# kylejckson/PaintFE

Hardware: AMD Instinct MI355X
Metric: Mpixels/sec: 8K 32-layer flatten + Gaussian sigma=16; HBM GB/s vs peak (higher is better)
Workload: dtype f32 (Gaussian leg: f16 taps x u8, f32 accumulate)

## Files before the change

paintfe_amd/csrc/k_flatten.hip:

```cpp
#include <algorithm>
#include <atomic>
#include <type_traits>
#include "k_common.h"
#include "pfx_kernels.h"

using namespace pfxk;

#include "k_blend.h"

typedef float pfx_v4f __attribute__((ext_vector_type(4)));
typedef int pfx_v4i __attribute__((ext_vector_type(4)));
__device__ pfx_v4f pfx_buffer_load_format_v4f32(pfx_v4i rsrc, int voffset, int soffset, int aux) __asm("llvm.amdgcn.raw.buffer.load.format.v4f32");
__device__ float pfx_buffer_load_format_f32(pfx_v4i rsrc, int voffset, int soffset, int aux) __asm("llvm.amdgcn.raw.buffer.load.format.f32");
__device__ void pfx_buffer_store_i32(int data, pfx_v4i rsrc, int voffset, int soffset, int aux) __asm("llvm.amdgcn.raw.buffer.store.i32");
__device__ void pfx_buffer_store_format_v4f32(pfx_v4f data, pfx_v4i rsrc, int voffset, int soffset, int aux) __asm("llvm.amdgcn.raw.buffer.store.format.v4f32");


namespace {


PFX_DEV uint32_t apply_conceal(uint32_t px, uint32_t conceal)
{
    if (conceal == 0u) return px;
    uint32_t a = ((px >> 24) * (255u - conceal)) / 255u;
// ... 417 lines not shown
                            const float a = pfx_buffer_load_format_f32(ra, (int)((base_px + o0 + 64u * j) * 4u), 0, 0);
                            const bool hit = C.kind[i] ? (a == 1.0f) : (a != 0.0f);
                            cls[j] = (cls[j] == 0u && hit) ? (uint32_t)(i + 1) : cls[j];
                            all_found = all_found && cls[j] != 0u;
                        }
                        done = __all(all_found);
                        st_reads += 1u;
                    }
                }
                uint32_t cnt[5] = {UPX, 0u, 0u, 0u, 0u};
#pragma unroll
                for (int i = 1; i <= 4; ++i)
#pragma unroll
                    for (int j = 0; j < PX; ++j) cnt[i] += (uint32_t)__popcll(__ballot(cls[j] >= (uint32_t)i));
                uint32_t cmin = 0;
#pragma unroll
                for (int i = 1; i <= 4; ++i) if (cnt[i] == UPX) cmin = (uint32_t)i;
                uint32_t lay[5] = {0u, C.layer[0], C.layer[1], C.layer[2], C.layer[3]};
                uint32_t s_u = 0;
#pragma unroll
                for (int i = 1; i <= 4; ++i) if (cmin == (uint32_t)i) s_u = lay[i];
                uint32_t best = 0, best_sav = 0, r = s_u;
#pragma unroll
                for (int i = 1; i <= 4; ++i) {
                    if ((uint32_t)i > cmin && (uint32_t)i <= C.n && cnt[i] * 10u >= UPX * 3u) {
                        const uint32_t sav = cnt[i] * (lay[i] - s_u);
                        if (sav > best_sav) { best_sav = sav; best = (uint32_t)i; r = lay[i]; }
                    }
                }
                if (best != 0u && q_cnt != 0u && q_r != r) { best = 0u; r = s_u; }
                if (probe) {
                    if (best != 0u || s_u != 0u) probe_fail = 0u;
                    else if (++probe_fail >= 2u) { probe_fail = 0u; skip_left = 14u; }
                }
#pragma unroll
                for (int j = 0; j < PX; ++j) acc_ring[(o0 + 64u * j) % RING] = 0u;
                if (best != 0u) {
                    st_cunits += 1u;
                    if (q_cnt == 0u) q_start = s_u; else q_start = min(q_start, s_u);
                    q_r = r;
#pragma unroll
                    for (int j = 0; j < PX; ++j) {
                        const bool early = cls[j] < best;
                        const uint64_t m = __ballot(early);
                        const uint32_t pre = __builtin_amdgcn_mbcnt_hi((uint32_t)(m >> 32), __builtin_amdgcn_mbcnt_lo((uint32_t)m, 0u));
                        if (early) q[(q_tail + pre) % QCAP] = (uint16_t)(o0 + 64u * j);
                        q_tail += (uint32_t)__popcll(m);
                    }
                }
                if (lane == 0) { rec[u % NREC][0] = r; rec[u % NREC][1] = best != 0u ? q_tail : 0u; }
                wave_lds_sync();
                cls_next = u + 1u;
                continue;
            }
            if (q_cnt == 0u) {
                if (lane == 0 && (C.stats & 1u)) {
                    atomicAdd(&g_dle_stats[0], st_rounds); atomicAdd(&g_dle_stats[1], st_rpx); atomicAdd(&g_dle_stats[2], st_rlay);
                    atomicAdd(&g_dle_stats[3], nat_next); atomicAdd(&g_dle_stats[4], st_nlay); atomicAdd(&g_dle_stats[5], st_reads);
                    atomicAdd(&g_dle_stats[6], st_cunits);
                }
                break;
            }
            run_queue = true;
        }

        int voff[PX];
        float acc[PX][4];
        uint32_t lb, le;
        if (run_queue) {
            const uint32_t m = min(q_cnt, UPX);
#pragma unroll
            for (int j = 0; j < PX; ++j) {
                const uint32_t k = 64u * j + lane;
                const uint32_t o = (uint32_t)q[(q_head + k) % QCAP];
                voff[j] = k < m ? (int)((base_px + o) * 4u) : (int)bytes;
                acc[j][0] = acc[j][1] = acc[j][2] = acc[j][3] = 0.0f;
            }
            lb = q_start; le = q_r;
            q_head += m;
            st_rounds += 1u; st_rpx += m; st_rlay += le - lb;
        } else {
            const uint32_t o0 = nat_next * UPX + lane;
#pragma unroll
            for (int j = 0; j < PX; ++j) {
                voff[j] = (int)((base_px + o0 + 64u * j) * 4u);
                const uint32_t p = acc_ring[(o0 + 64u * j) % RING];
                acc[j][0] = div255(ubyte0(p)); acc[j][1] = div255(ubyte1(p)); acc[j][2] = div255(ubyte2(p)); acc[j][3] = div255(ubyte3(p));
            }
            lb = nat_start; le = n_layers;
            st_nlay += le - lb;
        }
        dle_layers<PX, NB, AUX>(acc, layers, lb, le, bytes, voff, (C.stats & 2u) != 0u);
#pragma unroll
        for (int j = 0; j < PX; ++j) {
            const uint32_t px = (uint32_t)(acc[j][0] * 255.0f + 0.5f) | ((uint32_t)(acc[j][1] * 255.0f + 0.5f) << 8) |
                                ((uint32_t)(acc[j][2] * 255.0f + 0.5f) << 16) | ((uint32_t)(acc[j][3] * 255.0f + 0.5f) << 24);
            if (run_queue) { if (voff[j] != (int)bytes) acc_ring[((uint32_t)voff[j] / 4u - base_px) % RING] = px; }
            else pfx_buffer_store_i32((int)px, rs_dst, voff[j], 0, 0);
        }
        if (run_queue) wave_lds_sync();
        else nat_next += 1u;
    }
}


#ifndef PFX_SRT_GROUPS
#define PFX_SRT_GROUPS 1
#endif
#ifndef PFX_SRT_REDEAL
#define PFX_SRT_REDEAL 1
#endif
#ifndef PFX_SRT_TYPED_STORE
#define PFX_SRT_TYPED_STORE 0
#endif
#ifndef PFX_SRT_NATSTORE
#define PFX_SRT_NATSTORE 1
#endif
template <int PX>
PFX_DEV void stream_layer_groups(float (&acc)[PX][4], const float (&t)[PX][4], uint32_t mode, float opacity, uint32_t lead)
{
    const float amax = alpha_max<PX>(t);
#if PFX_TWO_STAGE
    if (__any(amax != 0.0f)) blend_layer_nx_two_stage<PX>(mode, acc, t, opacity, lead);
#elif PFX_SRT_GROUPS
    if (__any(amax != 0.0f)) blend_layer_nx_groups<PX>(mode, acc, t, opacity, lead);
#else
    if (__any(amax != 0.0f)) blend_layer_nx<PX>(mode, acc, t, opacity);
#endif
}

template <int PX, bool NOBLEND = false, bool TR = false>
PFX_DEV void srt_layers(float (&acc)[PX][4], const pfxk_layer_desc* __restrict__ layers, uint32_t lb, uint32_t le, uint32_t bytes, int (&voff)[PX],
                        uint32_t s1, uint32_t seg, float4* s_x, uint32_t* s_v, uint32_t& st_moves, unsigned long long* tr = nullptr)
{
    float t[2][PX][4];
    uint32_t m[2], o[2];
    const pfxk_layer_desc* nptr = layers + lb;
    pfxk_layer_desc nd = *nptr;
    uint32_t next_attempt = lb < s1 ? s1 : lb + 1u;
    uint32_t lead = 0u;
    bool recount = true;
    auto fetch = [&](auto SET) {
        constexpr int S = decltype(SET)::value;
        m[S] = nd.mode; o[S] = nd.adj_off;
        const pfx_v4i rs = make_rsrc_canonical(nd.pixels, bytes, PFX_RSRC_UNORM8X4);
#pragma unroll
        for (int j = 0; j < PX; ++j) {
            const pfx_v4f v = pfx_buffer_load_format_v4f32(rs, voff[j], 0, 0);
            t[S][j][0] = v.x; t[S][j][1] = v.y; t[S][j][2] = v.z; t[S][j][3] = v.w;
        }
        nptr += 1;
        nd = *nptr;
    };
    auto blend = [&](auto SET, uint32_t K) {
        constexpr int S = decltype(SET)::value;
        if (K < le) {
            unsigned long long c0 = 0, c1 = 0;
            if constexpr (TR) {
                c0 = __builtin_amdgcn_s_memtime();
                if constexpr (PX == 1) asm volatile("s_waitcnt vmcnt(1)" ::: "memory");
                else if constexpr (PX == 2) asm volatile("s_waitcnt vmcnt(2)" ::: "memory");
                else asm volatile("s_waitcnt vmcnt(3)" ::: "memory");
                c1 = __builtin_amdgcn_s_memtime();
                tr[0] += c1 - c0;
            }
            if constexpr (NOBLEND) {
#pragma unroll
                for (int j = 0; j < PX; ++j) { acc[j][0] += t[S][j][0]; acc[j][1] += t[S][j][1]; acc[j][2] += t[S][j][2]; acc[j][3] = t[S][j][3]; }
            } else if constexpr (PX == 1 && !PFX_TWO_STAGE) {
                stream_layer<1>(acc, t[S], m[S], __builtin_bit_cast(float, __builtin_amdgcn_readfirstlane(o[S])));
            } else {
                if (recount) { lead = count_lead<PX>(acc); recount = false; }
                stream_layer_groups<PX>(acc, t[S], m[S], __builtin_bit_cast(float, __builtin_amdgcn_readfirstlane(o[S])), lead);
                recount = m[S] == M_XOR || m[S] == M_OVERWRITE;
            }
            if constexpr (TR) {
                float sink = 0.0f;
#pragma unroll
                for (int j = 0; j < PX; ++j) sink += acc[j][0] + acc[j][3];
                asm volatile("" :: "v"(sink));
                tr[1] += __builtin_amdgcn_s_memtime() - c1;
            }
        }
    };
    auto redeal = [&](auto SET, uint32_t K) {
        constexpr int S = decltype(SET)::value;
#if !PFX_SRT_REDEAL
        return;
#endif
        if constexpr (PX == 1 || NOBLEND) return;
        if (K != next_attempt || K >= le) return;
        next_attempt = K + seg;
        uint64_t mo[PX];
        uint32_t co[PX], total_o = 0u, now = 0u;
        bool run = true;
#pragma unroll
        for (int j = 0; j < PX; ++j) {
            mo[j] = __ballot(acc[j][3] == 1.0f);
            co[j] = (uint32_t)__popcll(mo[j]);
            total_o += co[j];
            run = run && co[j] == 64u;
            now += run ? 1u : 0u;
        }
        lead = now; recount = false;
        if (total_o / 64u <= now) return;
        lead = total_o / 64u;
        const uint32_t lane = __builtin_amdgcn_mbcnt_hi(~0u, __builtin_amdgcn_mbcnt_lo(~0u, 0u));
        uint32_t slot[PX], pre_o = 0u, pre_n = total_o;
#pragma unroll
        for (int j = 0; j < PX; ++j) {
            const uint32_t rank_o = __builtin_amdgcn_mbcnt_hi((uint32_t)(mo[j] >> 32), __builtin_amdgcn_mbcnt_lo((uint32_t)mo[j], 0u));
            slot[j] = acc[j][3] == 1.0f ? pre_o + rank_o : pre_n + (lane - rank_o);
            pre_o += co[j]; pre_n += 64u - co[j];
        }
#pragma unroll
        for (int j = 0; j < PX; ++j) { s_x[slot[j]] = make_float4(acc[j][0], acc[j][1], acc[j][2], acc[j][3]); s_v[slot[j]] = (uint32_t)voff[j]; }
        wave_lds_sync();
#pragma unroll
        for (int j = 0; j < PX; ++j) {
            const float4 a = s_x[64u * j + lane];
            acc[j][0] = a.x; acc[j][1] = a.y; acc[j][2] = a.z; acc[j][3] = a.w;
            voff[j] = (int)s_v[64u * j + lane];
        }
        wave_lds_sync();
#pragma unroll
        for (int j = 0; j < PX; ++j) s_x[slot[j]] = make_float4(t[S][j][0], t[S][j][1], t[S][j][2], t[S][j][3]);
        wave_lds_sync();
#pragma unroll
        for (int j = 0; j < PX; ++j) {
            const float4 a = s_x[64u * j + lane];
            t[S][j][0] = a.x; t[S][j][1] = a.y; t[S][j][2] = a.z; t[S][j][3] = a.w;
        }
        wave_lds_sync();
        st_moves += 1u;
    };
    fetch(std::integral_constant<int, 0>{});
    for (uint32_t li = lb; li < le; li += 2) {
        fetch(std::integral_constant<int, 1>{}); blend(std::integral_constant<int, 0>{}, li); redeal(std::integral_constant<int, 1>{}, li + 1);
        fetch(std::integral_constant<int, 0>{}); blend(std::integral_constant<int, 1>{}, li + 1); redeal(std::integral_constant<int, 0>{}, li + 2);
    }
}

template <int NB, bool NOBLEND = false, bool TR = false>
PFX_DEV void srt_early(float (&acc)[1][4], const pfxk_layer_desc* __restrict__ layers, uint32_t lb, uint32_t le, uint32_t bytes, int voff, unsigned long long* tr = nullptr)
{
    static_assert(NB >= 2 && 2 * NB - 2 < PFXK_DESC_PAD, "descriptor padding");
    float t[NB][1][4];
    uint32_t m[NB], o[NB];
    const pfxk_layer_desc* nptr = layers + lb;
    pfxk_layer_desc nd = *nptr;
    uint32_t lead = 0u;
    bool recount = true;
    auto fetch = [&](auto SET) {
        constexpr int S = decltype(SET)::value;
        m[S] = nd.mode; o[S] = nd.adj_off;
        const pfx_v4i rs = make_rsrc_canonical(nd.pixels, bytes, PFX_RSRC_UNORM8X4);
        const pfx_v4f v = pfx_buffer_load_format_v4f32(rs, voff, 0, 0);
        t[S][0][0] = v.x; t[S][0][1] = v.y; t[S][0][2] = v.z; t[S][0][3] = v.w;
        nptr += 1;
        nd = *nptr;
    };
    auto blend = [&](auto SET, uint32_t K) {
        constexpr int S = decltype(SET)::value;
        if (K < le) {
            unsigned long long c0 = 0, c1 = 0;
            if constexpr (TR) {
                c0 = __builtin_amdgcn_s_memtime();
                asm volatile("s_waitcnt vmcnt(%0)" :: "n"(NB - 1) : "memory");
                c1 = __builtin_amdgcn_s_memtime();
                tr[0] += c1 - c0;
            }
            if constexpr (NOBLEND) { acc[0][0] += t[S][0][0]; acc[0][1] += t[S][0][1]; acc[0][2] += t[S][0][2]; acc[0][3] = t[S][0][3]; }
            else {
                if (recount) { lead = count_lead<1>(acc); recount = false; }
                stream_layer_groups<1>(acc, t[S], m[S], __builtin_bit_cast(float, __builtin_amdgcn_readfirstlane(o[S])), lead);
                recount = true;
            }
            if constexpr (TR) {
                const float sink = acc[0][0] + acc[0][3];
                asm volatile("" :: "v"(sink));
                tr[1] += __builtin_amdgcn_s_memtime() - c1;
            }
        }
    };
    auto seq = [&](auto self, auto I, uint32_t li) {
        constexpr int i = decltype(I)::value;
        if constexpr (i < NB) {
            fetch(std::integral_constant<int, (i + NB - 1) % NB>{});
            blend(std::integral_constant<int, i>{}, li + (uint32_t)i);
            self(self, std::integral_constant<int, i + 1>{}, li);
        }
    };
    auto pre = [&](auto self, auto I) {
        constexpr int i = decltype(I)::value;
        if constexpr (i < NB - 1) { fetch(std::integral_constant<int, i>{}); self(self, std::integral_constant<int, i + 1>{}); }
    };
    pre(pre, std::integral_constant<int, 0>{});
    for (uint32_t li = lb; li < le; li += (uint32_t)NB) seq(seq, std::integral_constant<int, 0>{}, li);
}
#ifndef PFX_EARLY_NB
#define PFX_EARLY_NB 2
#endif

struct dle_plan { uint32_t s1, seg; };

#ifndef PFX_SRT_PRIO
#define PFX_SRT_PRIO 0
#endif
#ifndef PFX_SRT_WAVES
#define PFX_SRT_WAVES 8
#endif
#if PFX_SRT_WAVES == 8
#define PFX_SRT_ATTR __attribute__((amdgpu_waves_per_eu(8, 8)))
#elif PFX_SRT_WAVES == 7
#define PFX_SRT_ATTR __attribute__((amdgpu_waves_per_eu(7, 7)))
#else
#define PFX_SRT_ATTR
#endif
template <int PX, bool NOBLEND = false, bool TR = false>
__global__ __launch_bounds__(64) PFX_SRT_ATTR void flatten_srt_kernel(const pfxk_layer_desc* __restrict__ layers, uint32_t n_layers, uint32_t n_px,
                                                                         uint8_t* __restrict__ dst, const pfxk_dle_cands C, const dle_sched SC,
                                                                         const dle_plan P)
{
    constexpr uint32_t UPX = 64u * PX;
    __shared__ float4 s_x[UPX];
    __shared__ uint32_t s_v[UPX];
    soft_d_fill(threadIdx.x, 64u);
    __syncthreads();
    const uint32_t lane = threadIdx.x & 63u;
    const uint32_t gw = __builtin_amdgcn_readfirstlane(blockIdx.x);
    const uint32_t units_total = (n_px + UPX - 1u) / UPX;
    uint32_t u0, U;
    if (gw < SC.wavesA) { U = SC.UA; u0 = gw * SC.UA; }
    else if (gw < SC.wavesA + SC.wavesB) { U = SC.UB; u0 = SC.wavesA * SC.UA + (gw - SC.wavesA) * SC.UB; }
    else { U = SC.UC; u0 = SC.wavesA * SC.UA + SC.wavesB * SC.UB + (gw - SC.wavesA - SC.wavesB) * SC.UC; }
    if (u0 >= units_total) return;
    const uint32_t nu = min(U, units_total - u0);
    const uint32_t base_px = u0 * UPX;
    const uint32_t bytes = n_px * 4u;
#if PFX_SRT_TYPED_STORE
    const pfx_v4i rs_acc = make_rsrc(dst, bytes, PFX_RSRC_UNORM8X4);
#else
    const pfx_v4i rs_dst = make_rsrc(dst, bytes, PFX_RSRC_RAW32);
#endif
    const uint32_t s1 = P.seg != 0u ? P.s1 : 0xFFFFFFFFu;
    uint32_t st_egroups = 0, st_elay = 0, st_nlay = 0, st_reads = 0, st_cunits = 0, st_moves = 0;
    uint32_t probe_fail = 0, skip_left = 0;
    unsigned long long tph[8] = {0, 0, 0, 0, 0, 0, 0, 0}, tc0 = 0;
    const unsigned long long t_birth = TR ? __builtin_amdgcn_s_memtime() : 0ull;
    for (uint32_t u = 0; u < nu; ++u) {
        if constexpr (TR) tc0 = __builtin_amdgcn_s_memtime();
        int voff[PX];
        float acc[PX][4];
#pragma unroll
        for (int j = 0; j < PX; ++j) {
            voff[j] = (int)((base_px + u * UPX + 64u * j + lane) * 4u);
            acc[j][0] = acc[j][1] = acc[j][2] = acc[j][3] = 0.0f;
        }
        uint32_t cls[PX];
#pragma unroll
        for (int j = 0; j < PX; ++j) cls[j] = 0u;
        const bool probe = skip_left == 0u;
        if (!probe) skip_left -= 1u;
        bool done = !probe;
#pragma unroll
        for (int i = 3; i >= 0; --i) {
            if ((uint32_t)i < C.n && !done) {
                const pfx_v4i ra = make_rsrc(layers[C.layer[i]].pixels, bytes, PFX_RSRC_ALPHA8);
                bool all_found = true;
#pragma unroll
                for (int j = 0; j < PX; ++j) {
                    const float a = pfx_buffer_load_format_f32(ra, voff[j], 0, 0);
                    const bool hit = C.kind[i] ? (a == 1.0f) : (a != 0.0f);
                    cls[j] = (cls[j] == 0u && hit) ? (uint32_t)(i + 1) : cls[j];
                    all_found = all_found && cls[j] != 0u;
                }
                done = __all(all_found);
                st_reads += 1u;
            }
        }
        uint32_t cn[5] = {UPX, 0u, 0u, 0u, 0u};
#pragma unroll
        for (int i = 1; i <= 4; ++i)
#pragma unroll
            for (int j = 0; j < PX; ++j) cn[i] += (uint32_t)__popcll(__ballot(cls[j] >= (uint32_t)i));
        uint32_t cmin = 0;
#pragma unroll
        for (int i = 1; i <= 4; ++i) if (cn[i] == UPX) cmin = (uint32_t)i;
        const uint32_t lay[5] = {0u, C.layer[0], C.layer[1], C.layer[2], C.layer[3]};
        uint32_t s_u = 0;
#pragma unroll
        for (int i = 1; i <= 4; ++i) if (cmin == (uint32_t)i) s_u = lay[i];
        uint32_t best = 0, best_sav = 0, r = s_u, eg = 0, cn_best = 0;
#pragma unroll
        for (int i = 1; i <= 4; ++i) {
            if ((uint32_t)i > cmin && (uint32_t)i <= C.n) {
                const uint32_t g = (UPX - cn[i] + 63u) / 64u;
                const uint32_t sav = ((uint32_t)PX - g) * (lay[i] - s_u);
                if (sav > best_sav) { best_sav = sav; best = (uint32_t)i; r = lay[i]; eg = g; cn_best = cn[i]; }
            }
        }
        if (probe) {
            if (best != 0u || s_u != 0u) probe_fail = 0u;
            else if (++probe_fail >= 2u) { probe_fail = 0u; skip_left = 14u; }
        }
        if constexpr (TR) { const unsigned long long c = __builtin_amdgcn_s_memtime(); tph[0] += c - tc0; tc0 = c; }
        if (best != 0u) {
            st_cunits += 1u;
            uint32_t pre_e = 0u, pre_l = UPX - cn_best;
#pragma unroll
            for (int j = 0; j < PX; ++j) {
                const bool early = cls[j] < best;
                const uint64_t m = __ballot(early);
                const uint32_t rank_e = __builtin_amdgcn_mbcnt_hi((uint32_t)(m >> 32), __builtin_amdgcn_mbcnt_lo((uint32_t)m, 0u));
                const uint32_t c = (uint32_t)__popcll(m);
                s_v[early ? pre_e + rank_e : pre_l + (lane - rank_e)] = (uint32_t)voff[j];
                pre_e += c; pre_l += 64u - c;
            }
            wave_lds_sync();
#pragma unroll
            for (int j = 0; j < PX; ++j) voff[j] = (int)s_v[64u * j + lane];
            wave_lds_sync();
            for (uint32_t g = 0; g < eg; ++g) {
                int v1[1];
                float a1[1][4] = {{0.0f, 0.0f, 0.0f, 0.0f}};
                v1[0] = voff[0];
#pragma unroll
                for (int j = 1; j < PX; ++j) v1[0] = g == (uint32_t)j ? voff[j] : v1[0];
                uint32_t none = 0u;
#if PFX_SRT_PRIO
                __builtin_amdgcn_s_setprio(PFX_SRT_PRIO & 3);
#endif
#if PFX_EARLY_NB > 0
                (void)none;
                srt_early<PFX_EARLY_NB, NOBLEND, TR>(a1, layers, s_u, r, bytes, v1[0], tph + 4);
#else
                srt_layers<1, NOBLEND, TR>(a1, layers, s_u, r, bytes, v1, 0xFFFFFFFFu, 0u, s_x, s_v, none, tph + 4);
#endif
#pragma unroll
                for (int j = 0; j < PX; ++j)
                    if (g == (uint32_t)j) { acc[j][0] = a1[0][0]; acc[j][1] = a1[0][1]; acc[j][2] = a1[0][2]; acc[j][3] = a1[0][3]; }
            }
            st_egroups += eg; st_elay += eg * (r - s_u);
        }
        st_nlay += n_layers - r;
        const uint32_t moves_before = st_moves;
        if constexpr (TR) { const unsigned long long c = __builtin_amdgcn_s_memtime(); tph[1] += c - tc0; tc0 = c; }
#if PFX_SRT_PRIO
        __builtin_amdgcn_s_setprio((PFX_SRT_PRIO >> 2) & 3);
#endif
        srt_layers<PX, NOBLEND, TR>(acc, layers, r, n_layers, bytes, voff, s1, P.seg, s_x, s_v, st_moves, tph + 6);
        if constexpr (TR) { const unsigned long long c = __builtin_amdgcn_s_memtime(); tph[2] += c - tc0; tc0 = c; }
        if (PFX_SRT_NATSTORE && (best != 0u || st_moves != moves_before)) {
            const uint32_t ub = (base_px + u * UPX) * 4u;
#pragma unroll
            for (int j = 0; j < PX; ++j) s_x[((uint32_t)voff[j] - ub) >> 2] = make_float4(acc[j][0], acc[j][1], acc[j][2], acc[j][3]);
            wave_lds_sync();
#pragma unroll
            for (int j = 0; j < PX; ++j) {
                const float4 a = s_x[64u * j + lane];
                acc[j][0] = a.x; acc[j][1] = a.y; acc[j][2] = a.z; acc[j][3] = a.w;
                voff[j] = (int)(ub + (64u * j + lane) * 4u);
            }
            wave_lds_sync();
        }
#pragma unroll
        for (int j = 0; j < PX; ++j) {
#if PFX_SRT_TYPED_STORE
            pfx_v4f v; v.x = acc[j][0]; v.y = acc[j][1]; v.z = acc[j][2]; v.w = acc[j][3];
            pfx_buffer_store_format_v4f32(v, rs_acc, voff[j], 0, 0);
#else
            uint32_t px = 0u;
#pragma unroll
            for (int c = 0; c < 4; ++c) px = __builtin_amdgcn_cvt_pk_u8_f32(acc[j][c] * 255.0f, c, px);
            pfx_buffer_store_i32((int)px, rs_dst, voff[j], 0, 0);
#endif
        }
        if constexpr (TR) { const unsigned long long c = __builtin_amdgcn_s_memtime(); tph[3] += c - tc0; tc0 = c; }
    }
    if constexpr (TR) {
        if (lane == 0) {
#pragma unroll
            for (int i = 0; i < 8; ++i) atomicAdd(&g_dle_stats[8 + i], tph[i]);
            atomicAdd(&g_dle_stats[0], __builtin_amdgcn_s_memtime() - t_birth);
            atomicAdd(&g_dle_stats[1], 1ull);
        }
        return;
    }
    if (lane == 0 && (C.stats & 1u)) {
        atomicAdd(&g_dle_stats[0], st_egroups); atomicAdd(&g_dle_stats[1], st_egroups * 64u); atomicAdd(&g_dle_stats[2], st_elay);
        atomicAdd(&g_dle_stats[3], nu); atomicAdd(&g_dle_stats[4], st_nlay); atomicAdd(&g_dle_stats[5], st_reads);
        atomicAdd(&g_dle_stats[6], st_cunits); atomicAdd(&g_dle_stats[7], st_moves);
    }
}

__global__ __launch_bounds__(1024) void dle_probe_kernel(const pfxk_layer_desc* __restrict__ layers, uint32_t cand_layer, uint32_t cand_kind, uint32_t n_px,
                                                         uint32_t* __restrict__ verdict_pinned, uint32_t tag)
{
    __shared__ uint32_t s_cnt;
    if (threadIdx.x == 0) s_cnt = 0u;
    __syncthreads();
    const uint32_t lane = threadIdx.x & 63u, wave = threadIdx.x >> 6;
    const uint32_t units = (n_px + 191u) / 192u, bytes = n_px * 4u;
    const pfx_v4i ra = make_rsrc(layers[cand_layer].pixels, bytes, PFX_RSRC_ALPHA8);
    uint32_t good = 0u;
#pragma unroll 4
    for (uint32_t k = 0; k < 16u; ++k) {
        const uint32_t u = (uint32_t)(((uint64_t)(wave * 16u + k) * units) / 256u);
        bool all_hit = true;
#pragma unroll
        for (uint32_t j = 0; j < 3u; ++j) {
            const uint32_t px = u * 192u + 64u * j + lane;
            const float a = pfx_buffer_load_format_f32(ra, (int)(px * 4u), 0, 0);
            all_hit = all_hit && (px >= n_px || (cand_kind ? (a == 1.0f) : (a != 0.0f)));
        }
        good += __all(all_hit) ? 1u : 0u;
    }
    if (lane == 0) atomicAdd(&s_cnt, good);
    __syncthreads();
    if (threadIdx.x == 0) *verdict_pinned = tag | (s_cnt * 2u >= 256u ? 0x80000000u : 0u);
}

__global__ __launch_bounds__(256) void unorm_store_check_kernel(uint8_t* __restrict__ scratch , unsigned long long* out)
{
    const uint32_t k = threadIdx.x;
    const float bn = div255((float)k);
    const pfx_v4i rs = make_rsrc(scratch, 1024u, PFX_RSRC_UNORM8X4);
    pfx_v4f v; v.x = bn; v.y = div255((float)(255u - k)); v.z = div255((float)((k * 7u) & 255u)); v.w = bn;
    pfx_buffer_store_format_v4f32(v, rs, (int)(k * 4u), 0, 0);
    __syncthreads();
    const uint32_t raw = reinterpret_cast<const volatile uint32_t*>(scratch)[k];
    const uint32_t want = k | ((255u - k) << 8) | (((k * 7u) & 255u) << 16) | (k << 24);
    const pfx_v4f b = pfx_buffer_load_format_v4f32(rs, (int)(k * 4u), 0, 0);
    const bool ok = raw == want && __builtin_bit_cast(uint32_t, b.x) == __builtin_bit_cast(uint32_t, v.x) &&
                    __builtin_bit_cast(uint32_t, b.y) == __builtin_bit_cast(uint32_t, v.y) &&
                    __builtin_bit_cast(uint32_t, b.z) == __builtin_bit_cast(uint32_t, v.z) && __builtin_bit_cast(uint32_t, b.w) == __builtin_bit_cast(uint32_t, v.w);
    if (!ok) atomicAdd(out, 1ull);
}

std::atomic<int> g_dle_stats_on{0}, g_dle_cfg{0}, g_dle_sched{1}, g_dle_fracA{75}, g_dle_fracB{20};
std::atomic<int> g_dle_units{0};
std::atomic<int> g_dle_kernel{0};
std::atomic<int> g_dle_s1{-1}, g_dle_s2{-1};
std::atomic<int> g_flatten_variant{0};

__global__ __launch_bounds__(256) void chunk_alpha_flags_kernel(const uint8_t* __restrict__ px, uint32_t w, uint32_t h, uint32_t cx0, uint32_t cy0,
                                                                uint32_t ncx, uint8_t* __restrict__ flags)
{
    const uint32_t cxn = (w + 63u) / 64u;
    const uint32_t cx = cx0 + blockIdx.x % ncx, cy = cy0 + blockIdx.x / ncx;
    const uint32_t bx = cx * 64u, by = cy * 64u;
    const uint32_t cw = min(64u, w - bx), ch = min(64u, h - by);
    int not_opaque = 0, has_zero = 0;
    for (uint32_t i = threadIdx.x; i < cw * ch; i += blockDim.x) {
        const uint32_t a = px[((size_t)(by + i / cw) * w + bx + i % cw) * 4 + 3];
        not_opaque |= a != 255u;
        has_zero |= a == 0u;
    }
    const int any_no = __syncthreads_or(not_opaque), any_zero = __syncthreads_or(has_zero);
    if (threadIdx.x == 0) flags[cy * cxn + cx] = (uint8_t)((any_no ? 0u : 1u) | (any_zero ? 0u : 2u));
}

__global__ __launch_bounds__(256) void chunk_start_kernel(const uint8_t* const* __restrict__ flags, const uint8_t* __restrict__ want, uint32_t n_layers,
                                                          uint32_t n_chunks, uint8_t* __restrict__ start, uint32_t* __restrict__ useful, uint32_t tag)
{
    const uint32_t c = blockIdx.x * blockDim.x + threadIdx.x;
    if (c >= n_chunks) return;
    uint32_t s = 0u;
    for (uint32_t k = 1; k < n_layers; ++k)
        if (want[k] && flags[k] && (flags[k][c] & want[k])) s = k;
    start[c] = (uint8_t)min(s, 254u);
    if (s != 0u && useful) *useful = tag;
}

__global__ __launch_bounds__(256) void chunk_active_kernel(const pfxk_layer_desc* __restrict__ layers, uint32_t n_layers,
                                                           uint32_t w, uint32_t h, uint8_t* __restrict__ chunk_active,
                                                           const uint8_t* __restrict__ preview_present)
{
    const uint32_t cxn = (w + 63u) / 64u;
    const uint32_t cx = blockIdx.x % cxn, cy = blockIdx.x / cxn;
    const uint32_t bx = cx * 64u, by = cy * 64u;
    const uint32_t cw = min(64u, w - bx), ch = min(64u, h - by);
    int any = preview_present ? (preview_present[blockIdx.x] != 0) : 0;
    for (uint32_t li = 0; li < n_layers && !any; ++li) {
        const pfxk_layer_desc L = layers[li];
        if (L.kind != PFXK_LAYER_RASTER || !L.pixels) continue;
        int mine = 0;
        for (uint32_t i = threadIdx.x; i < cw * ch; i += blockDim.x) {
            uint32_t lx = i % cw, ly = i / cw;
            mine |= L.pixels[((size_t)(by + ly) * w + bx + lx) * 4 + 3] != 0;
        }
        any = __syncthreads_or(mine);
    }
    if (threadIdx.x == 0) chunk_active[blockIdx.x] = (uint8_t)(any != 0);
}

template <bool F>
__global__ __launch_bounds__(256) void blend_arrays_kernel(const uint32_t* __restrict__ base, const uint32_t* __restrict__ top,
                                                           uint32_t* __restrict__ dst, size_t n, uint32_t mode, float opacity)
{
    for (size_t i = (size_t)blockIdx.x * blockDim.x + threadIdx.x; i < n; i += (size_t)gridDim.x * blockDim.x) {
        const uint32_t b = base[i];
        float acc[4][4];
        acc[0][0] = ubyte0(b); acc[0][1] = ubyte1(b); acc[0][2] = ubyte2(b); acc[0][3] = ubyte3(b);
#pragma unroll
        for (int p = 1; p < 4; ++p) acc[p][0] = acc[p][1] = acc[p][2] = acc[p][3] = 0.0f;
        const uint32_t t[4] = {top[i], 0u, 0u, 0u};
        blend4_dispatch<F>(mode, acc, t, opacity, rs_clamp(opacity, 0.0f, 1.0f));
        dst[i] = pack_rgba(acc[0][0], acc[0][1], acc[0][2], acc[0][3]);
    }
}

__global__ __launch_bounds__(256) void brush_commit_kernel(uint32_t* __restrict__ layer, const uint32_t* __restrict__ preview,
                                                           const uint8_t* __restrict__ selection, size_t n, uint32_t mode,
                                                           int is_eraser)
{
    for (size_t i = (size_t)blockIdx.x * blockDim.x + threadIdx.x; i < n; i += (size_t)gridDim.x * blockDim.x) {
        if (selection && selection[i] == 0) continue;
        const uint32_t pp = preview[i];
        if ((pp >> 24) == 0u) continue;
        const uint32_t lp = layer[i];
        if (is_eraser) {
            const float mask_strength = div255(ubyte3(pp));
            const float current_a = div255(ubyte3(lp));
            const float new_a = __builtin_fmaxf(current_a * (1.0f - mask_strength), 0.0f);
            layer[i] = (lp & 0x00ffffffu) | ((uint32_t)trunc_u8f(new_a * 255.0f) << 24);
        } else {
            float acc[4][4];
            acc[0][0] = ubyte0(lp); acc[0][1] = ubyte1(lp); acc[0][2] = ubyte2(lp); acc[0][3] = ubyte3(lp);
#pragma unroll
            for (int p = 1; p < 4; ++p) acc[p][0] = acc[p][1] = acc[p][2] = acc[p][3] = 0.0f;
            const uint32_t t[4] = {pp, 0u, 0u, 0u};
            blend4_dispatch<true>(mode, acc, t, 1.0f, 1.0f);
            layer[i] = pack_rgba(acc[0][0], acc[0][1], acc[0][2], acc[0][3]);
        }
    }
}

__global__ __launch_bounds__(256) void rdiv_check_kernel(uint64_t seed, uint32_t iters, unsigned long long* out)
{
    uint64_t s = seed + ((uint64_t)blockIdx.x * blockDim.x + threadIdx.x) * 0x9E3779B97F4A7C15ull;
    unsigned long long bad = 0;
    for (uint32_t i = 0; i < iters; ++i) {
        s = s * 6364136223846793005ull + 1442695040888963407ull;
        const uint32_t a = (uint32_t)(s >> 33), b = (uint32_t)(s >> 7);
        const float n = ((a & 0xC0u) == 0u) ? 0.0f : __builtin_bit_cast(float, ((a >> 8) & 0x007fffffu) | ((127u - (a & 31u)) << 23));
        const float d = __builtin_bit_cast(float, (b & 0x007fffffu) | ((127u - ((b >> 23) % 49u)) << 23));
        const float q_ref = n / d;
        const float q_fast = rdiv_apply(rdiv_prepare(d), n);
        bad += (__builtin_bit_cast(uint32_t, q_ref) != __builtin_bit_cast(uint32_t, q_fast));
    }
    if (bad) atomicAdd(out, bad);
}

__global__ __launch_bounds__(256) void round_pack_check_kernel(unsigned long long* out)
{
    const uint64_t tid = (uint64_t)blockIdx.x * blockDim.x + threadIdx.x, nth = (uint64_t)gridDim.x * blockDim.x;
    unsigned long long bad = 0, bad_snan = 0;
    for (uint64_t b = tid; b < (1ull << 32); b += nth) {
        const uint32_t bits = (uint32_t)b;
        const float v = __builtin_bit_cast(float, bits);
        const uint32_t fast = pack_round_rgba(v, 0.0f, 0.0f, 0.0f) & 0xffu;
        const uint32_t ref = (v != v) ? 0u : (uint32_t)round_u8f(v);
        if (fast != ref) {
            const bool snan = (bits & 0x7f800000u) == 0x7f800000u && (bits & 0x007fffffu) != 0u && !(bits & 0x00400000u);
            if (snan) ++bad_snan; else ++bad;
        }
    }
    if (bad) atomicAdd(out, bad);
    if (bad_snan) atomicAdd(out + 1, bad_snan);
}

}

extern "C" void pfxk_flatten_set_variant(int v) { g_flatten_variant = v; }
extern "C" hipError_t pfxk_chunk_alpha_flags(hipStream_t s, const uint8_t* d_px, uint32_t w, uint32_t h, uint32_t cx0, uint32_t cy0, uint32_t ncx, uint32_t ncy,
                                             uint8_t* d_flags)
{
    if (ncx == 0 || ncy == 0) return hipSuccess;
    chunk_alpha_flags_kernel<<<ncx * ncy, 256, 0, s>>>(d_px, w, h, cx0, cy0, ncx, d_flags);
    return hipGetLastError();
}
extern "C" hipError_t pfxk_chunk_start(hipStream_t s, const uint8_t* const* d_flag_ptrs, const uint8_t* d_want, uint32_t n_layers, uint32_t n_chunks,
                                       uint8_t* d_start, uint32_t* useful_pinned, uint32_t tag)
{
    if (n_chunks == 0) return hipSuccess;
    chunk_start_kernel<<<(n_chunks + 255) / 256, 256, 0, s>>>(d_flag_ptrs, d_want, n_layers, n_chunks, d_start, useful_pinned, tag);
    return hipGetLastError();
}
extern "C" hipError_t pfxk_flatten_dle_stats(unsigned long long* out16, int reset)
{
    hipError_t e = hipSuccess;
    if (out16) e = hipMemcpyFromSymbol(out16, HIP_SYMBOL(g_dle_stats), 16 * sizeof(unsigned long long));
    if (e == hipSuccess && reset) {
        const unsigned long long z[16] = {};
        e = hipMemcpyToSymbol(HIP_SYMBOL(g_dle_stats), z, sizeof z);
    }
    return e;
}
extern "C" void pfxk_flatten_set_dle(int units_per_wave, int ring_log2)
{
    if (units_per_wave >= 0) g_dle_units = units_per_wave;
    (void)ring_log2;
}
extern "C" void pfxk_flatten_set_dle_dev(int stats_on, int cfg)
{
    if (stats_on >= 0) g_dle_stats_on = stats_on;
    if (cfg >= 0) g_dle_cfg = cfg;
}
extern "C" void pfxk_flatten_set_dle_sched(int sched, int fracA, int fracB)
{
    if (sched >= 0) g_dle_sched = sched;
    if (fracA >= 0 && fracA <= 100) g_dle_fracA = fracA;
    if (fracB >= 0 && fracB <= 100 - g_dle_fracA) g_dle_fracB = fracB;
}
extern "C" void pfxk_flatten_set_dle_plan(int kernel, int s1, int s2)
{
    if (kernel >= 0) g_dle_kernel = kernel;
    if (s1 >= -1) g_dle_s1 = s1;
    if (s2 >= -1) g_dle_s2 = s2;
}
extern "C" hipError_t pfxk_dle_probe(hipStream_t s, const pfxk_layer_desc* d_layers, uint32_t cand_layer, uint32_t cand_kind, uint32_t n_px, uint32_t* verdict_pinned,
                                     uint32_t tag)
{
    dle_probe_kernel<<<1, 1024, 0, s>>>(d_layers, cand_layer, cand_kind, n_px, verdict_pinned, tag);
    return hipGetLastError();
}
extern "C" hipError_t pfxk_unorm_store_check(hipStream_t s, uint8_t* d_scratch1k, unsigned long long* d_out)
{
    unorm_store_check_kernel<<<1, 256, 0, s>>>(d_scratch1k, d_out);
    return hipGetLastError();
}
extern "C" hipError_t pfxk_round_pack_check(hipStream_t s, unsigned long long* d_out)
{
    round_pack_check_kernel<<<4096, 256, 0, s>>>(d_out);
    return hipGetLastError();
}

extern "C" hipError_t pfxk_rdiv_check(hipStream_t s, uint64_t seed, uint32_t blocks, uint32_t iters, unsigned long long* d_out)
{
    rdiv_check_kernel<<<blocks, 256, 0, s>>>(seed, iters, d_out);
    return hipGetLastError();
}

extern "C" hipError_t pfxk_blend_arrays(hipStream_t s, const uint8_t* d_base, const uint8_t* d_top, uint8_t* d_dst,
                                        size_t n_px, uint32_t mode, float opacity, int fast_div)
{
    if (n_px == 0) return hipSuccess;
    size_t blocks = (n_px + 255) / 256;
    if (blocks > 8192) blocks = 8192;
    if (fast_div)
        blend_arrays_kernel<true><<<(uint32_t)blocks, 256, 0, s>>>((const uint32_t*)d_base, (const uint32_t*)d_top,
                                                                   (uint32_t*)d_dst, n_px, mode, opacity);
// ... 117 lines not shown
```

Before: 29480.

## Pipeline layer fetches across units and prefetch next unit's alpha probe

Adds software-pipelined variants of the early-group and main layer-streaming loops. They double-buffer layer texels and read descriptors through the constant address space. During the last layer of the current unit, the top candidate layer's alpha for the next unit is prefetched, so the probe load latency overlaps with blending. This raises register pressure from the extra double buffers and adds complexity in the redeal and slot paths, which could lower occupancy under the fixed waves-per-EU setting.

```diff
diff --git a/paintfe_amd/csrc/k_flatten.hip b/paintfe_amd/csrc/k_flatten.hip
--- a/paintfe_amd/csrc/k_flatten.hip
+++ b/paintfe_amd/csrc/k_flatten.hip
@@ -743,6 +743,193 @@
 #define PFX_EARLY_NB 2
 #endif
 
+#ifndef PFX_SRT_PIPE
+#define PFX_SRT_PIPE 1
+#endif
+#ifndef PFX_SRT_PIPE_PARTS
+#define PFX_SRT_PIPE_PARTS 2
+#endif
+
+typedef const __attribute__((address_space(4))) pfxk_layer_desc* pfx_desc_cptr;
+PFX_DEV pfx_desc_cptr desc_const(const pfxk_layer_desc* p) { return (pfx_desc_cptr)p; }
+PFX_DEV void desc_read(pfxk_layer_desc& d, pfx_desc_cptr p) { d.pixels = p->pixels; d.mode = p->mode; d.adj_off = p->adj_off; }
+
+template <int PX, bool NOBLEND, class Slot>
+PFX_DEV void srt_layers_pipe(float (&acc)[PX][4], float (&t)[2][PX][4], const pfxk_layer_desc* __restrict__ layers, uint32_t lb, uint32_t le, uint32_t bytes,
+                             int (&voff)[PX], uint32_t s1, uint32_t seg, float4* s_x, uint32_t* s_v, uint32_t& st_moves, bool inflight, Slot&& slot)
+{
+    uint32_t m[2], o[2];
+    pfx_desc_cptr nptr = desc_const(layers + lb);
+    pfxk_layer_desc nd;
+    desc_read(nd, nptr);
+    uint32_t next_attempt = lb < s1 ? s1 : lb + 1u;
+    uint32_t lead = 0u;
+    bool recount = true;
+    auto fetch = [&](auto SET) {
+        constexpr int S = decltype(SET)::value;
+        m[S] = nd.mode; o[S] = nd.adj_off;
+        const pfx_v4i rs = make_rsrc_canonical(nd.pixels, bytes, PFX_RSRC_UNORM8X4);
+#pragma unroll
+        for (int j = 0; j < PX; ++j) {
+            const pfx_v4f v = pfx_buffer_load_format_v4f32(rs, voff[j], 0, 0);
+            t[S][j][0] = v.x; t[S][j][1] = v.y; t[S][j][2] = v.z; t[S][j][3] = v.w;
+        }
+        nptr += 1;
+        desc_read(nd, nptr);
+    };
+    auto blend = [&](auto SET) {
+        constexpr int S = decltype(SET)::value;
+        if constexpr (NOBLEND) {
+#pragma unroll
+            for (int j = 0; j < PX; ++j) { acc[j][0] += t[S][j][0]; acc[j][1] += t[S][j][1]; acc[j][2] += t[S][j][2]; acc[j][3] = t[S][j][3]; }
+        } else if constexpr (PX == 1 && !PFX_TWO_STAGE) {
+            stream_layer<1>(acc, t[S], m[S], __builtin_bit_cast(float, __builtin_amdgcn_readfirstlane(o[S])));
+        } else {
+            if (recount) { lead = count_lead<PX>(acc); recount = false; }
+            stream_layer_groups<PX>(acc, t[S], m[S], __builtin_bit_cast(float, __builtin_amdgcn_readfirstlane(o[S])), lead);
+            recount = m[S] == M_XOR || m[S] == M_OVERWRITE;
+        }
+    };
+    auto redeal = [&](auto SET, uint32_t K) {
+        constexpr int S = decltype(SET)::value;
+#if !PFX_SRT_REDEAL
+        return;
+#endif
+        if constexpr (PX == 1 || NOBLEND) return;
+        if (K != next_attempt) return;
+        next_attempt = K + seg;
+        uint64_t mo[PX];
+        uint32_t co[PX], total_o = 0u, now = 0u;
+        bool run = true;
+#pragma unroll
+        for (int j = 0; j < PX; ++j) {
+            mo[j] = __ballot(acc[j][3] == 1.0f);
+            co[j] = (uint32_t)__popcll(mo[j]);
+            total_o += co[j];
+            run = run && co[j] == 64u;
+            now += run ? 1u : 0u;
+        }
+        lead = now; recount = false;
+        if (total_o / 64u <= now) return;
+        lead = total_o / 64u;
+        const uint32_t lane = __builtin_amdgcn_mbcnt_hi(~0u, __builtin_amdgcn_mbcnt_lo(~0u, 0u));
+        uint32_t slot[PX], pre_o = 0u, pre_n = total_o;
+#pragma unroll
+        for (int j = 0; j < PX; ++j) {
+            const uint32_t rank_o = __builtin_amdgcn_mbcnt_hi((uint32_t)(mo[j] >> 32), __builtin_amdgcn_mbcnt_lo((uint32_t)mo[j], 0u));
+            slot[j] = acc[j][3] == 1.0f ? pre_o + rank_o : pre_n + (lane - rank_o);
+            pre_o += co[j]; pre_n += 64u - co[j];
+        }
+#pragma unroll
+        for (int j = 0; j < PX; ++j) { s_x[slot[j]] = make_float4(acc[j][0], acc[j][1], acc[j][2], acc[j][3]); s_v[slot[j]] = (uint32_t)voff[j]; }
+        wave_lds_sync();
+#pragma unroll
+        for (int j = 0; j < PX; ++j) {
+            const float4 a = s_x[64u * j + lane];
+            acc[j][0] = a.x; acc[j][1] = a.y; acc[j][2] = a.z; acc[j][3] = a.w;
+            voff[j] = (int)s_v[64u * j + lane];
+        }
+        wave_lds_sync();
+#pragma unroll
+        for (int j = 0; j < PX; ++j) s_x[slot[j]] = make_float4(t[S][j][0], t[S][j][1], t[S][j][2], t[S][j][3]);
+        wave_lds_sync();
+#pragma unroll
+        for (int j = 0; j < PX; ++j) {
+            const float4 a = s_x[64u * j + lane];
+            t[S][j][0] = a.x; t[S][j][1] = a.y; t[S][j][2] = a.z; t[S][j][3] = a.w;
+        }
+        wave_lds_sync();
+        st_moves += 1u;
+    };
+    if (inflight) { m[0] = nd.mode; o[0] = nd.adj_off; nptr += 1; desc_read(nd, nptr); }
+    else fetch(std::integral_constant<int, 0>{});
+    uint32_t li = lb;
+    for (; li + 2u < le; li += 2) {
+        fetch(std::integral_constant<int, 1>{}); blend(std::integral_constant<int, 0>{}); redeal(std::integral_constant<int, 1>{}, li + 1);
+        fetch(std::integral_constant<int, 0>{}); blend(std::integral_constant<int, 1>{}); redeal(std::integral_constant<int, 0>{}, li + 2);
+    }
+    if (li + 1u < le) {
+        fetch(std::integral_constant<int, 1>{}); blend(std::integral_constant<int, 0>{}); redeal(std::integral_constant<int, 1>{}, li + 1);
+        slot(); blend(std::integral_constant<int, 1>{});
+    } else { slot(); blend(std::integral_constant<int, 0>{}); }
+}
+
+template <int PX, bool NOBLEND>
+PFX_DEV void srt_early_pipe(float (&acc)[PX][4], float (&tn)[2][PX][4], const pfxk_layer_desc* __restrict__ layers, uint32_t lb, uint32_t le, uint32_t bytes,
+                            const int (&voff)[PX], uint32_t eg)
+{
+    float t[2][1][4], a1[1][4];
+    uint32_t m[2], o[2];
+    pfx_desc_cptr nptr = desc_const(layers + lb);
+    pfxk_layer_desc nd;
+    desc_read(nd, nptr);
+    uint32_t lead = 0u;
+    bool recount = true;
+    int v = voff[0];
+    auto fetch = [&](auto SET) {
+        constexpr int S = decltype(SET)::value;
+        m[S] = nd.mode; o[S] = nd.adj_off;
+        const pfx_v4i rs = make_rsrc_canonical(nd.pixels, bytes, PFX_RSRC_UNORM8X4);
+        const pfx_v4f x = pfx_buffer_load_format_v4f32(rs, v, 0, 0);
+        t[S][0][0] = x.x; t[S][0][1] = x.y; t[S][0][2] = x.z; t[S][0][3] = x.w;
+        nptr += 1;
+        desc_read(nd, nptr);
+    };
+    auto blend = [&](auto SET) {
+        constexpr int S = decltype(SET)::value;
+        if constexpr (NOBLEND) { a1[0][0] += t[S][0][0]; a1[0][1] += t[S][0][1]; a1[0][2] += t[S][0][2]; a1[0][3] = t[S][0][3]; }
+        else {
+            if (recount) { lead = count_lead<1>(a1); recount = false; }
+            stream_layer_groups<1>(a1, t[S], m[S], __builtin_bit_cast(float, __builtin_amdgcn_readfirstlane(o[S])), lead);
+            recount = true;
+        }
+    };
+    auto slot = [&](auto LAST, auto FREE, uint32_t g) {
+        if constexpr (decltype(LAST)::value) {
+            if constexpr (PFX_SRT_PIPE_PARTS >= 3) {
+                const pfx_v4i rs = make_rsrc_canonical(nd.pixels, bytes, PFX_RSRC_UNORM8X4);
+#pragma unroll
+                for (int j = 0; j < PX; ++j) {
+                    const pfx_v4f x = pfx_buffer_load_format_v4f32(rs, voff[j], 0, 0);
+                    tn[0][j][0] = x.x; tn[0][j][1] = x.y; tn[0][j][2] = x.z; tn[0][j][3] = x.w;
+                }
+            }
+        } else {
+#pragma unroll
+            for (int j = 1; j < PX; ++j) v = g + 1u == (uint32_t)j ? voff[j] : v;
+            nptr = desc_const(layers + lb);
+            desc_read(nd, nptr);
+            fetch(FREE);
+        }
+    };
+    auto group = [&](auto LAST, uint32_t g) {
+        a1[0][0] = a1[0][1] = a1[0][2] = a1[0][3] = 0.0f;
+        recount = true;
+        bool moved = false;
+        uint32_t li = lb;
+        for (; li + 2u < le; li += 2) {
+            fetch(std::integral_constant<int, 1>{}); blend(std::integral_constant<int, 0>{});
+            fetch(std::integral_constant<int, 0>{}); blend(std::integral_constant<int, 1>{});
+        }
+        if (li + 1u < le) {
+            fetch(std::integral_constant<int, 1>{}); blend(std::integral_constant<int, 0>{});
+            slot(LAST, std::integral_constant<int, 0>{}, g); blend(std::integral_constant<int, 1>{});
+        } else { slot(LAST, std::integral_constant<int, 1>{}, g); blend(std::integral_constant<int, 0>{}); moved = true; }
+        if (!decltype(LAST)::value && moved) {
+#pragma unroll
+            for (int c = 0; c < 4; ++c) t[0][0][c] = t[1][0][c];
+            m[0] = m[1]; o[0] = o[1];
+        }
+#pragma unroll
+        for (int j = 0; j < PX; ++j)
+#pragma unroll
+            for (int c = 0; c < 4; ++c) acc[j][c] = g == (uint32_t)j ? a1[0][c] : acc[j][c];
+    };
+    fetch(std::integral_constant<int, 0>{});
+    for (uint32_t g = 0; g + 1u < eg; ++g) group(std::false_type{}, g);
+    group(std::true_type{}, eg - 1u);
+}
+
 struct dle_plan { uint32_t s1, seg; };
 
 #ifndef PFX_SRT_PRIO
@@ -789,6 +976,17 @@
     uint32_t probe_fail = 0, skip_left = 0;
     unsigned long long tph[8] = {0, 0, 0, 0, 0, 0, 0, 0}, tc0 = 0;
     const unsigned long long t_birth = TR ? __builtin_amdgcn_s_memtime() : 0ull;
+    constexpr bool PIPE = PFX_SRT_PIPE != 0 && !TR && PFX_EARLY_NB == 2;
+    float pa[PX];
+    auto alpha_ahead = [&](uint32_t unit, bool wanted) {
+        const uint32_t top_layer = C.n >= 4u ? C.layer[3] : (C.n == 3u ? C.layer[2] : (C.n == 2u ? C.layer[1] : C.layer[0]));
+        const pfx_v4i ra = make_rsrc(desc_const(layers + top_layer)->pixels, wanted ? bytes : 0u, PFX_RSRC_ALPHA8);
+        const uint32_t l = __builtin_amdgcn_mbcnt_hi(~0u, __builtin_amdgcn_mbcnt_lo(~0u, 0u));
+        const int vo = (int)((base_px + unit * UPX + l) * 4u);
+#pragma unroll
+        for (int j = 0; j < PX; ++j) pa[j] = pfx_buffer_load_format_f32(ra, vo + j * 256, 0, 0);
+    };
+    if constexpr (PIPE) alpha_ahead(0u, true);
     for (uint32_t u = 0; u < nu; ++u) {
         if constexpr (TR) tc0 = __builtin_amdgcn_s_memtime();
         int voff[PX];
@@ -807,12 +1005,19 @@
 #pragma unroll
         for (int i = 3; i >= 0; --i) {
             if ((uint32_t)i < C.n && !done) {
-                const pfx_v4i ra = make_rsrc(layers[C.layer[i]].pixels, bytes, PFX_RSRC_ALPHA8);
+                float a[PX];
+                if (PIPE && (uint32_t)i + 1u == C.n) {
+#pragma unroll
+                    for (int j = 0; j < PX; ++j) a[j] = pa[j];
+                } else {
+                    const pfx_v4i ra = make_rsrc(layers[C.layer[i]].pixels, bytes, PFX_RSRC_ALPHA8);
+#pragma unroll
+                    for (int j = 0; j < PX; ++j) a[j] = pfx_buffer_load_format_f32(ra, voff[j], 0, 0);
+                }
                 bool all_found = true;
 #pragma unroll
                 for (int j = 0; j < PX; ++j) {
-                    const float a = pfx_buffer_load_format_f32(ra, voff[j], 0, 0);
-                    const bool hit = C.kind[i] ? (a == 1.0f) : (a != 0.0f);
+                    const bool hit = C.kind[i] ? (a[j] == 1.0f) : (a[j] != 0.0f);
                     cls[j] = (cls[j] == 0u && hit) ? (uint32_t)(i + 1) : cls[j];
                     all_found = all_found && cls[j] != 0u;
                 }
@@ -846,6 +1051,9 @@
             else if (++probe_fail >= 2u) { probe_fail = 0u; skip_left = 14u; }
         }
         if constexpr (TR) { const unsigned long long c = __builtin_amdgcn_s_memtime(); tph[0] += c - tc0; tc0 = c; }
+        [[maybe_unused]] float tnat[2][PX][4];
+        [[maybe_unused]] bool nat_inflight = false;
+        [[maybe_unused]] const bool issue_next = u + 1u < nu && skip_left == 0u;
         if (best != 0u) {
             st_cunits += 1u;
             uint32_t pre_e = 0u, pre_l = UPX - cn_best;
@@ -862,6 +1070,13 @@
 #pragma unroll
             for (int j = 0; j < PX; ++j) voff[j] = (int)s_v[64u * j + lane];
             wave_lds_sync();
+            if constexpr (PIPE && PFX_SRT_PIPE_PARTS >= 2) {
+#if PFX_SRT_PRIO
+                __builtin_amdgcn_s_setprio(PFX_SRT_PRIO & 3);
+#endif
+                srt_early_pipe<PX, NOBLEND>(acc, tnat, layers, s_u, r, bytes, voff, eg);
+                nat_inflight = PFX_SRT_PIPE_PARTS >= 3;
+            } else
             for (uint32_t g = 0; g < eg; ++g) {
                 int v1[1];
                 float a1[1][4] = {{0.0f, 0.0f, 0.0f, 0.0f}};
@@ -890,6 +1105,10 @@
 #if PFX_SRT_PRIO
         __builtin_amdgcn_s_setprio((PFX_SRT_PRIO >> 2) & 3);
 #endif
+        if constexpr (PIPE) {
+            srt_layers_pipe<PX, NOBLEND>(acc, tnat, layers, r, n_layers, bytes, voff, s1, P.seg, s_x, s_v, st_moves, nat_inflight,
+                                         [&]() { alpha_ahead(u + 1u, issue_next); });
+        } else
         srt_layers<PX, NOBLEND, TR>(acc, layers, r, n_layers, bytes, voff, s1, P.seg, s_x, s_v, st_moves, tph + 6);
         if constexpr (TR) { const unsigned long long c = __builtin_amdgcn_s_memtime(); tph[2] += c - tc0; tc0 = c; }
         if (PFX_SRT_NATSTORE && (best != 0u || st_moves != moves_before)) {
```

Result: faster. 29820, median of 6 (+1.1%).
